# Starfish-develop/Starfish

Hardware: AMD Instinct MI355X
Metric: log-likelihood evals/sec, 4096-pixel order, batch=128 walkers (higher is better)
Workload: dtype f64; 1 GPU; cfg2: synthetic single order N_pix=4096, 8 eigenspectra, M=27, N_f=8192, 1 global + 1 local kernel, all 13 parameters thawed, batch=128 walkers per GPU; global_batch=128, units_per_gpu=128, parallelism=(order x walker) units sharded x1, one process per GPU, no data-path collective

## Files before the change

### starfish_amd/csrc/sf_chol_seq.h

```cpp
#pragma once
#include "sf_chol_host.h"
#include "sf_chol_diag.h"
#include "sf_chol_panel.h"
#include "sf_chol_wide.h"

static int sf_check_front_pad(int fp, int n) {
    if (fp != 0 && (fp != 64 || n % GT != 64)) {
        sf_set_error("potrf: front pad %d does not fit n = %d", fp, n);
        return SF_EINVAL;
    }
    return SF_OK;
}

template <class Args>
static void sf_park(Args& g, const sf_potrf_scratch& ws) {
    g.Sout = ws.T;
    g.sS = ws.sT;
    g.ldS = SF_LDT;
}
static double sf_slab_rows(int n, int row0, int nslab, int step) {
    double rows = 0.0;
    for (int i = 0; i < nslab; ++i) {
        const int r0 = row0 + i * step * GT;
        rows += (n - r0 < GT) ? n - r0 : GT;
    }
    return rows;
}
static int sf_check_grid(long long nblk) {
    if (nblk > 0x7fffffffLL) {
        sf_set_error("panel grid too large");
        return SF_EINVAL;
    }
    return SF_OK;
}

static int sf_panel_split(int k0, int pw, int fp, long long nblk) {
    return pw > 0 ? sf_split_policy(nblk, (k0 > fp ? k0 - fp : 0) / GK) : 1;
}
static int sf_panel_step(sf_panel_args g, const sf_potrf_scratch& ws, int k0, int pw, int row0, int nslab, int step, const double* Wt,
                         bool to_scratch, hipStream_t st, int region, int phase) {
    const int n = g.n, fp = g.fp, batch = ws.batch;
    g.k0 = k0;
    g.pw = pw;
    g.row0 = row0;
    g.nslab = nslab;
    g.slab_step = step;
    g.Wt = Wt;
    g.sW = ws.sW;
    if (to_scratch) {
        sf_park(g, ws);
        g.prio = 1;
    }
    const long long nblk = (long long)nslab * batch;
    SF_TRY(sf_check_grid(nblk));
    const double rows = sf_slab_rows(n, row0, nslab, step);
    const double flops_main = 2.0 * (k0 > fp ? k0 - fp : 0) * rows * pw * batch;
    const double flops_epi = (rows * pw * (double)pw + (double)GT * rows * pw) * batch;
    const int nk = (k0 > fp ? k0 - fp : 0) / GK;
    const int S = sf_panel_split(k0, pw, fp, nblk);
    void* tok;
    if (S > 1) {
        g.ksplit = S;
        g.kchunk = (nk + S - 1) / S;
        g.part = ws.part + (size_t)region * sf_split_region_tiles() * (GT * GT);
        if (phase != 2) {
            sf_prof_gemm_begin(st, flops_main, &tok);
            hipLaunchKernelGGL((k_chol_panel<false, 1>), dim3((unsigned)(nblk * S)), dim3(512), 0, st, g);
            sf_prof_gemm_end(tok);
        }
        if (phase != 1) {
            sf_prof_gemm_begin(st, flops_epi, &tok);
            if (g.rhs)
                hipLaunchKernelGGL((k_chol_panel<true, 2>), dim3((unsigned)nblk), dim3(512), 0, st, g);
            else
                hipLaunchKernelGGL((k_chol_panel<false, 2>), dim3((unsigned)nblk), dim3(512), 0, st, g);
            sf_prof_gemm_end(tok);
        }
    } else {
        sf_prof_gemm_begin(st, flops_main + flops_epi, &tok);
        if (g.rhs)
            hipLaunchKernelGGL((k_chol_panel<true, 0>), dim3((unsigned)nblk), dim3(512), 0, st, g);
        else
            hipLaunchKernelGGL((k_chol_panel<false, 0>), dim3((unsigned)nblk), dim3(512), 0, st, g);
        sf_prof_gemm_end(tok);
    }
    SF_LAUNCH_CHECK();
    return SF_OK;
}

struct sf_wide_stamps {
#ifdef SF_TUNING
    long long* t = nullptr;
    int n = 0, k[64];
#endif
};
#ifdef SF_TUNING
static int sf_wide_stamps_begin(sf_wide_stamps& w) {
    if (SF_TUNE_FLAG("SF_WIDE_STAMPS")) {
        SF_HIP(hipHostMalloc((void**)&w.t, sizeof(long long) * 16 * 64));
        for (int i = 0; i < 16 * 64; ++i) w.t[i] = 0;
    }
    return SF_OK;
}
static void sf_wide_stamps_report(sf_wide_stamps& w, hipStream_t s) {
    if (!w.t) return;
    (void)hipStreamSynchronize(s);
    fprintf(stderr, "wide launches, workgroup grid/2: k nslab | prologue | K loop | solve 1 | 2b | solve 2 | store + rhs | S load + step 4 | S store + drain | total (us)\n");
    for (int i = 0; i < w.n; ++i) {
        const long long* t = w.t + 16 * i;
        fprintf(stderr, "%2d %2d |", w.k[i] / 1000, w.k[i] % 1000);
        const int seg[8][2] = {{0, 1}, {1, 2}, {2, 3}, {3, 4}, {4, 5}, {5, 6}, {6, 7}, {7, 8}};
        for (auto& sg : seg) fprintf(stderr, " %7.1f |", (t[sg[1]] - t[sg[0]]) / 100.0);
        fprintf(stderr, " %7.1f\n", (t[8] - t[0]) / 100.0);
    }
    (void)hipHostFree(w.t);
}
#else
static int sf_wide_stamps_begin(sf_wide_stamps&) { return SF_OK; }
static void sf_wide_stamps_report(sf_wide_stamps&, hipStream_t) {}
#endif

static int sf_panel_step_w(sf_panelw_args g, const sf_potrf_scratch& ws, int k, int slab0, int nslab, int step, bool park, hipStream_t st,
                           sf_wide_stamps& stamps) {
    const int n = g.n, fp = g.fp, batch = ws.batch;
    g.k0 = k * GT;
    g.row0 = slab0 * GT;
    g.nslab = nslab;
    g.slab_step = step;
    g.Wt0 = ws.Wslot(k);
    g.Wt1 = ws.Wslot(k + 1);
    g.sW = ws.sW;
    if (park) sf_park(g, ws);
    const long long nblk = (long long)nslab * batch;
    SF_TRY(sf_check_grid(nblk));
#ifdef SF_TUNING
    if (stamps.t && stamps.n < 64) {
        stamps.k[stamps.n] = k * 1000 + nslab;
        g.stamps = stamps.t + 16 * stamps.n++;
    }
#endif
    const double rows = sf_slab_rows(n, g.row0, nslab, step);
    const double kk = g.k0 > fp ? g.k0 - fp : 0;
    const double flops = (2.0 * kk * rows * GT + 2.0 * (kk + GT) * rows * GT + 2.0 * (rows * GT * (double)GT + (double)GT * rows * GT)) * batch;
    void* tok;
    sf_prof_gemm_begin(st, flops, &tok);
    if (g.rhs)
        hipLaunchKernelGGL(k_chol_panel_w<true>, dim3((unsigned)nblk), dim3(1024), SF_PANELW_LDS, st, g);
    else
        hipLaunchKernelGGL(k_chol_panel_w<false>, dim3((unsigned)nblk), dim3(1024), SF_PANELW_LDS, st, g);
    sf_prof_gemm_end(tok);
    SF_LAUNCH_CHECK();
    return SF_OK;
}

static int sf_diag_step(const sf_potrf_scratch& ws, double* A, int lda, int64_t stride, double* rhs, int ldr, int* info, int n, int k,
                        double* Wt, int fp, hipStream_t st) {
    const int k0 = k * GT;
    const int pw = (n - k0 < GT) ? n - k0 : GT;
    return sf_launch_diag128(ws.T, ws.sT, pw, info, k0 - fp, rhs ? rhs + k0 : nullptr, ldr, A + (int64_t)k0 * lda + k0, lda, stride, Wt,
                             ws.sW, ws.batch, st, k == 0 ? fp : 0);
}

struct sf_narrow_events {
    hipEvent_t d, rest[2];
};
static int sf_narrow_step(const sf_panel_args& base, const sf_potrf_scratch& ws, sf_exec* ex, int* info, int k, double* Wt, hipStream_t c,
                          const hipStream_t gs[2], const hipEvent_t last[2], hipEvent_t* e_top, sf_narrow_events* ev) {
    const int n = base.n, fp = base.fp, nt = (n + GT - 1) / GT;
    const int k0 = k * GT;
    const int pw = (n - k0 < GT) ? n - k0 : GT;
    *ev = {};
    SF_TRY(sf_diag_step(ws, base.C, base.lda, base.sC, base.rhs, base.ldr, info, n, k, Wt, fp, c));
    if (k + 1 >= nt) return SF_OK;
    SF_TRY(sf_exec_event(ex, &ev->d));
    SF_HIP(hipEventRecord(ev->d, c));
    const int gk = (k + 1) & 1;
    if (e_top && sf_panel_split(k0, pw, fp, ws.batch) > 1) {
        if (*e_top) SF_HIP(hipStreamWaitEvent(gs[gk], *e_top, 0));
        SF_TRY(sf_panel_step(base, ws, k0, pw, (k + 1) * GT, 1, 1, Wt, true, gs[gk], 0, 1));
        hipEvent_t e_part;
        SF_TRY(sf_exec_event(ex, &e_part));
        SF_HIP(hipEventRecord(e_part, gs[gk]));
        SF_HIP(hipStreamWaitEvent(c, e_part, 0));
        SF_TRY(sf_panel_step(base, ws, k0, pw, (k + 1) * GT, 1, 1, Wt, true, c, 0, 2));
    } else {
        if (last[gk]) SF_HIP(hipStreamWaitEvent(c, last[gk], 0));
        SF_TRY(sf_panel_step(base, ws, k0, pw, (k + 1) * GT, 1, 1, Wt, true, c, 0, 0));
    }
    if (e_top) {
        SF_TRY(sf_exec_event(ex, e_top));
        SF_HIP(hipEventRecord(*e_top, c));
    }
    for (int g = 0; g < 2; ++g) {
        const int first = k + 2 + (((k + 2) & 1) != g);
        if (first >= nt) continue;
        const int cnt = (nt - 1 - first) / 2 + 1;
        SF_HIP(hipStreamWaitEvent(gs[g], ev->d, 0));
        SF_TRY(sf_panel_step(base, ws, k0, pw, first * GT, cnt, 2, Wt, false, gs[g], 1 + g, 0));
        SF_TRY(sf_exec_event(ex, &ev->rest[g]));
        SF_HIP(hipEventRecord(ev->rest[g], gs[g]));
    }
    return SF_OK;
}

static int sf_launch_potrf_v2(double* A, int n, int lda, int64_t stride, int* info, const sf_potrf_scratch& ws, double* rhs,
                              int ldr, hipStream_t s, const sf_gen_args* gen, sf_exec* ex, int fp) {
    const int batch = ws.batch;
    SF_HIP(hipMemsetAsync(info, 0, sizeof(int) * (size_t)batch, s));
    SF_TRY(sf_exec_prepare(ex));
    constexpr int G = 2;
    hipStream_t c = ex->side;
    const hipStream_t gs[G] = {s, ex->grp[0]};
    SF_TRY(sf_exec_fork(ex, s, {c, gs[1]}));

    const sf_panel_args base = sf_panel_frame<sf_panel_args>(A, n, lda, stride, rhs, ldr, gen, fp);
    const int nt = (n + GT - 1) / GT;
    SF_TRY(sf_panel_step(base, ws, 0, 0, 0, 1, 1, nullptr, true, c, 0, 0));
    hipEvent_t e_epi = nullptr;
    hipEvent_t e_rest[G] = {};
    hipEvent_t e_rest_prev[G] = {};
    for (int k = 0; k < nt; ++k) {
        for (int g = 0; g < G; ++g)
            if (e_rest_prev[g]) SF_HIP(hipStreamWaitEvent(c, e_rest_prev[g], 0));
        sf_narrow_events ev;
        SF_TRY(sf_narrow_step(base, ws, ex, info, k, ws.Wbuf(k & 1), c, gs, e_rest, &e_epi, &ev));
        for (int g = 0; g < G; ++g) {
            e_rest_prev[g] = e_rest[g];
            if (ev.rest[g]) e_rest[g] = ev.rest[g];
        }
    }
    SF_TRY(sf_exec_join(ex, s, c, {e_rest[1]}));
    return SF_OK;
}

static int sf_launch_potrf_v3(double* A, int n, int lda, int64_t stride, int* info, const sf_potrf_scratch& ws, double* rhs,
                              int ldr, hipStream_t s, const sf_gen_args* gen, sf_exec* ex, bool half, int fp) {
    const int batch = ws.batch;
    static sf_dev_once attr_once;
    SF_CHECK(sf_lds_limit_once(&attr_once, 160 * 1024, {(const void*)k_chol_panel_w<true>, (const void*)k_chol_panel_w<false>}));
    SF_HIP(hipMemsetAsync(info, 0, sizeof(int) * (size_t)batch, s));
    SF_TRY(sf_exec_prepare(ex));
    hipStream_t c = ex->side, xa = ex->side;
    SF_TRY(sf_exec_fork(ex, s, {c, xa, ex->grp[0]}));
    const int nt = (n + GT - 1) / GT;

    const sf_panel_args base = sf_panel_frame<sf_panel_args>(A, n, lda, stride, rhs, ldr, gen, fp);
    const sf_panelw_args wbase = sf_panel_frame<sf_panelw_args>(A, n, lda, stride, rhs, ldr, gen, fp);
    sf_wide_stamps stamps;
    SF_TRY(sf_wide_stamps_begin(stamps));
    auto diag = [&](int k) -> int { return sf_diag_step(ws, A, lda, stride, rhs, ldr, info, n, k, ws.Wslot(k), fp, c); };

    SF_TRY(sf_panel_step(base, ws, 0, 0, 0, 1, 1, nullptr, true, c, 0, 0));
    const hipStream_t bs[2] = {s, ex->grp[0]};
    hipEvent_t e_A = nullptr;
    hipEvent_t e_last[2] = {nullptr, nullptr};
    std::vector<hipEvent_t> readers[4];
    auto wait_readers = [&](int slot) -> int {
        for (hipEvent_t e : readers[slot]) SF_HIP(hipStreamWaitEvent(c, e, 0));
        readers[slot].clear();
        return SF_OK;
    };
    int k = 0;
    for (; k < nt; k += 2) {
        if (k + 2 >= nt) break;
        if (half && k >= (nt / 4) * 2 && k > 0) break;
        if (e_A) SF_HIP(hipStreamWaitEvent(c, e_A, 0));
        SF_TRY(wait_readers(k & 3));
        SF_TRY(diag(k));
        SF_TRY(sf_panel_step(base, ws, k * GT, GT, (k + 1) * GT, 1, 1, ws.Wslot(k), true, c, 0, 0));
        SF_TRY(wait_readers((k + 1) & 3));
        SF_TRY(diag(k + 1));
        hipEvent_t e_chain;
        SF_TRY(sf_exec_event(ex, &e_chain));
        SF_HIP(hipEventRecord(e_chain, c));
        const int na = (nt - (k + 2) < 2) ? nt - (k + 2) : 2;
        SF_HIP(hipStreamWaitEvent(xa, e_chain, 0));
        for (int g = 0; g < 2; ++g)
            if (e_last[g]) SF_HIP(hipStreamWaitEvent(xa, e_last[g], 0));
        SF_TRY(sf_panel_step_w(wbase, ws, k, k + 2, na, 1, true, xa, stamps));
        SF_TRY(sf_exec_event(ex, &e_A));
        SF_HIP(hipEventRecord(e_A, xa));
        readers[k & 3].push_back(e_A);
        readers[(k + 1) & 3].push_back(e_A);
        for (int g = 0; g < 2; ++g) {
            const int first = k + 4 + g;
            if (first >= nt) continue;
            const int cnt = (nt - 1 - first) / 2 + 1;
            SF_HIP(hipStreamWaitEvent(bs[g], e_chain, 0));
            SF_TRY(sf_panel_step_w(wbase, ws, k, first, cnt, 2, false, bs[g], stamps));
            SF_TRY(sf_exec_event(ex, &e_last[g]));
            SF_HIP(hipEventRecord(e_last[g], bs[g]));
            readers[k & 3].push_back(e_last[g]);
            readers[(k + 1) & 3].push_back(e_last[g]);
        }
    }
    for (; k < nt; ++k) {
        if (e_A) {
            SF_HIP(hipStreamWaitEvent(c, e_A, 0));
            for (int g = 0; g < 2; ++g) SF_HIP(hipStreamWaitEvent(bs[g], e_A, 0));
            e_A = nullptr;
        }
        SF_TRY(wait_readers(k & 3));
        sf_narrow_events ev;
        SF_TRY(sf_narrow_step(base, ws, ex, info, k, ws.Wslot(k), c, bs, e_last, nullptr, &ev));
        for (int g = 0; g < 2; ++g)
            if (ev.rest[g]) {
                e_last[g] = ev.rest[g];
                readers[k & 3].push_back(ev.rest[g]);
            }
    }
    SF_TRY(sf_exec_join(ex, s, c, {e_A, e_last[1]}));
    sf_wide_stamps_report(stamps, s);
    return SF_OK;
}
```

### starfish_amd/csrc/sf_chol_wide.h

```cpp
#pragma once
#include "sf_device.h"
#include "sf_chol_tile.h"
#include "sf_chol_panel.h"

#define WST (3 * GT * GK)
static constexpr size_t SF_PANELW_LDS = (3 * WST + 4 * GT) * sizeof(double);
struct sf_panelw_args {
    double* C;
    int64_t sC;
    int lda, n;
    int k0;
    int row0, nslab;
    int slab_step;
    const double* Wt0;
    const double* Wt1;
    int64_t sW;
    double* rhs;
    int ldr;
    double* Sout;
    int64_t sS;
    int ldS;
    const double* genY;
    const unsigned char* tilemap;
    int64_t sY;
    int ldy, mpad, nt128;
    int fp;
#ifdef SF_TUNING
    long long* stamps;
#endif
};
#ifdef SF_TUNING
#define SF_W_STAMP(i) do { if (g.stamps && blockIdx.x == gridDim.x / 2 && threadIdx.x == 0) g.stamps[i] = wall_clock64(); } while (0)
#else
#define SF_W_STAMP(i)
#endif

template <bool RHS>
__device__ __forceinline__ void sf_panelw_body(const sf_panelw_args& g, const int id, double* __restrict__ smw, const int tid) {
    constexpr int TM = 2, TN = 4;
    double* red = smw + 3 * WST;

    const int b = id / g.nslab;
    const int sl = id - b * g.nslab;
    const int row0 = g.row0 + sl * g.slab_step * GT;
    const int rows_here = min(GT, g.n - row0);
    const int k0 = g.k0;
    const int cfp = k0 == 0 ? g.fp : 0;

    const int lane = tid & 63;
    const int w = __builtin_amdgcn_readfirstlane(tid >> 6);
    const int wm = w & 3, wn = w >> 2;
    const int l15 = lane & 15, lq = lane >> 4;
    double* Cb = g.C + (int64_t)b * g.sC;
#define WBC(ni) ((((ni) >> 1) * GT) + wn * 32 + (((ni)&1) * 16))
    const bool wave_live = wm * 32 < rows_here;

    sf_d4 acc[TM][TN];
    SF_W_STAMP(0);
    {
        typedef __attribute__((address_space(3))) void* lds_ptr;
        const unsigned lds0 = (unsigned)(size_t)(lds_ptr)smw;
        const int grow = lane >> 3, gpos = lane & 7;
        unsigned soff[3];
        const double* sbase = sf_uniform_ptr(Cb + g.fp);
#pragma unroll
        for (int j = 0; j < 3; ++j) {
            const int G = 3 * w + j;
            const bool isA = G < 16;
            const int r = (isA ? G : G - 16) * 8 + grow;
            const int c = gpos ^ sf_swz(r);
            soff[j] = (unsigned)(((int64_t)(isA ? row0 + min(r, rows_here - 1) : k0 + r) * g.lda + 2 * c) * 8);
        }
        auto glds16 = [&](const double* sb, unsigned voff, unsigned lds_dst) {
            unsigned keep;
            asm volatile("s_mov_b32 %0, m0\n\ts_mov_b32 m0, %3\n\ts_nop 0\n\tglobal_load_lds_dwordx4 %1, %2\n\ts_mov_b32 m0, %0"
                         : "=&s"(keep)
                         : "v"(voff), "s"(sb), "s"(lds_dst)
                         : "memory");
        };
        auto gload = [&](int kt, int stage) {
#pragma unroll
            for (int j = 0; j < 3; ++j) glds16(sf_uniform_ptr(sbase + kt * GK), soff[j], lds0 + (unsigned)(stage * WST * 8 + (3 * w + j) * 1024));
        };
        auto gwait = [&]() { asm volatile("s_waitcnt vmcnt(0)" ::: "memory"); };
        const int nk = max(k0 - g.fp, 0) / GK;
        if (nk > 0) gload(0, 0);
        if (nk > 1) gload(1, 1);

        bool gen_half[2] = {false, false};
        if (g.tilemap) {
            const unsigned char* tm = g.tilemap + (int64_t)b * g.nt128 * g.nt128 + (row0 / GT) * g.nt128 + k0 / GT;
            gen_half[0] = !tm[0];
            gen_half[1] = !tm[1];
        }
#pragma unroll
        for (int hf = 0; hf < 2; ++hf) {
            if (gen_half[hf]) {
                const double* Yb = g.genY + (int64_t)b * g.sY;
                const int gr = row0 + wm * 32 + l15;
                const int gc = k0 + hf * GT + wn * 32 + l15;
#pragma unroll
                for (int mi = 0; mi < TM; ++mi)
#pragma unroll
                    for (int nn = 0; nn < 2; ++nn) acc[mi][2 * hf + nn] = (sf_d4){0.0, 0.0, 0.0, 0.0};
                for (int kk = 0; kk < g.mpad; kk += 8) {
                    double ya[2][TM], yb[2][2];
#pragma unroll
                    for (int u = 0; u < 2; ++u) {
                        const double* yk = Yb + (int64_t)(min(kk + 4 * u, g.mpad - 4) + lq) * g.ldy;
#pragma unroll
                        for (int i = 0; i < TM; ++i) ya[u][i] = yk[min(gr + i * 16, g.ldy + g.fp - 1)];
#pragma unroll
                        for (int i = 0; i < 2; ++i) yb[u][i] = gc + i * 16 >= cfp ? yk[min(gc + i * 16, g.ldy + g.fp - 1)] : 0.0;
                    }
#pragma unroll
                    for (int u = 0; u < 2; ++u) {
                        if (kk + 4 * u >= g.mpad) break;
#pragma unroll
                        for (int mi = 0; mi < TM; ++mi)
#pragma unroll
                            for (int nn = 0; nn < 2; ++nn)
                                acc[mi][2 * hf + nn] = __builtin_amdgcn_mfma_f64_16x16x4f64(ya[u][mi], yb[u][nn], acc[mi][2 * hf + nn], 0, 0, 0);
                    }
                }
            } else {
                const double* Cin = Cb + (int64_t)row0 * g.lda + k0;
#pragma unroll
                for (int mi = 0; mi < TM; ++mi)
#pragma unroll
                    for (int nn = 0; nn < 2; ++nn) {
                        const int col = WBC(2 * hf + nn) + l15;
#pragma unroll
                        for (int r = 0; r < 4; ++r) {
                            const int row = wm * 32 + mi * 16 + lq + 4 * r;
                            acc[mi][2 * hf + nn][r] = (row < rows_here && col >= cfp) ? Cin[(int64_t)row * g.lda + col] : 0.0;
                        }
                    }
            }
        }
        gwait();
        __syncthreads();
#pragma unroll
        for (int mi = 0; mi < TM; ++mi)
#pragma unroll
            for (int ni = 0; ni < TN; ++ni)
#pragma unroll
                for (int r = 0; r < 4; ++r) asm volatile("" : "+v"(acc[mi][ni][r]));
        SF_W_STAMP(1);

        const int sw = sf_swz(l15);
        const int e0 = 2 * ((2 * lq) ^ sw), e1 = 2 * ((2 * lq + 1) ^ sw);
        const int arow = (wm * 32 + l15) * GK, brow = (GT + wn * 32 + l15) * GK;
        auto frag = [&](int stage, int h, double2(&a)[TM], double2(&bb)[TN]) {
            const double* S = smw + stage * WST + (h ? e1 : e0);
#pragma unroll
            for (int i = 0; i < TM; ++i) a[i] = *(const double2*)(S + arow + i * 16 * GK);
#pragma unroll
            for (int i = 0; i < TN; ++i) bb[i] = *(const double2*)(S + brow + ((i >> 1) * GT + (i & 1) * 16) * GK);
        };
        auto mfma_part = [&](const double2(&a)[TM], const double2(&bb)[TN], auto lo_t, auto hi_t) {
            constexpr int lo = decltype(lo_t)::value, hi = decltype(hi_t)::value;
#pragma unroll
            for (int i = lo; i < hi; ++i) {
                const int y = i >> 3, mi = (i >> 2) & 1, ni = i & 3;
                acc[mi][ni] = __builtin_amdgcn_mfma_f64_16x16x4f64(y ? a[mi].y : a[mi].x, y ? bb[ni].y : bb[ni].x, acc[mi][ni], 0, 0, 1);
            }
        };
        typedef std::integral_constant<int, 0> I0;
        typedef std::integral_constant<int, 8> I8;
        typedef std::integral_constant<int, 16> I16;
        double2 a0[TM], b0[TN], a1[TM], b1[TN];
        int s0 = 0, s1 = 1, s2 = 2;
        if (nk > 0 && wave_live) frag(0, 0, a0, b0);
        for (int kt = 0; kt < nk; ++kt) {
            if (wave_live) {
                __builtin_amdgcn_s_setprio(1);
                mfma_part(a0, b0, I0(), I8());
                __builtin_amdgcn_s_setprio(0);
            }
            if (kt + 2 < nk) gload(kt + 2, s2);
            if (wave_live) {
                frag(s0, 1, a1, b1);
                __builtin_amdgcn_s_setprio(1);
                mfma_part(a0, b0, I8(), I16());
                __builtin_amdgcn_s_setprio(0);
                if (kt + 1 < nk) frag(s1, 0, a0, b0);
                __builtin_amdgcn_s_setprio(1);
                mfma_part(a1, b1, I0(), I16());
                __builtin_amdgcn_s_setprio(0);
            }
            gwait();
            __syncthreads();
            const int t = s0;
            s0 = s1;
            s1 = s2;
            s2 = t;
        }
    }

    double* Ach0 = smw;
    double* Bs = smw + 2 * GT * CLD;
    const int lr = tid >> 3, lc = (tid & 7) * 2;
    auto w_rows = [&](const double* Wt) { return Wt + (int64_t)b * g.sW + (int64_t)lr * SF_LDT + lc; };
    auto solve = [&](const double* Wt, double2 rw, auto nbtag) {
        constexpr int NB = decltype(nbtag)::value;
        const double* Wp = w_rows(Wt);
        int buf = 0;
#pragma unroll
        for (int sbi = 0; sbi < 8; ++sbi) {
            const int sb = 7 - sbi;
            double* Ach = Ach0 + ((sb >> 1) & 1) * (GT * CLD);
            if (sb == 7 && NB != 0) __syncthreads();
            if (sb & 1) {
                if (wn == (sb >> 1)) {
#pragma unroll
                    for (int nn = 0; nn < 2; ++nn)
#pragma unroll
                        for (int mi = 0; mi < TM; ++mi) {
#pragma unroll
                            for (int r = 0; r < 4; ++r)
                                Ach[(wm * 32 + mi * 16 + lq + 4 * r) * CLD + nn * 16 + l15] = acc[mi][NB + nn][r];
                            acc[mi][NB + nn] = (sf_d4){0.0, 0.0, 0.0, 0.0};
                        }
                }
            }
            {
                double* pb = Bs + buf * (GT * GLD) + lr * GLD + lc;
                pb[0] = rw.x;
                pb[1] = rw.y;
            }
            __syncthreads();
            if (sb > 0) rw = *(const double2*)(Wp + (sb - 1) * 16);
            if (sb <= 2 * wn + 1 && wave_live) {
                const double* Ab = Ach + (wm * 32 + l15) * CLD + (sb & 1) * 16 + lq;
                const double* Bb = Bs + buf * (GT * GLD) + (wn * 32 + l15) * GLD + lq;
#pragma unroll
                for (int ks = 0; ks < 4; ++ks) {
                    double a[TM], bb[2];
#pragma unroll
                    for (int i = 0; i < TM; ++i) a[i] = Ab[i * 16 * CLD + ks * 4];
#pragma unroll
                    for (int i = 0; i < 2; ++i) bb[i] = Bb[i * 16 * GLD + ks * 4];
#pragma unroll
                    for (int mi = 0; mi < TM; ++mi)
#pragma unroll
                        for (int nn = 0; nn < 2; ++nn)
                            acc[mi][NB + nn] = __builtin_amdgcn_mfma_f64_16x16x4f64(a[mi], bb[nn], acc[mi][NB + nn], 0, 0, 0);
                }
            }
            buf ^= 1;
        }
    };
    double2 rw0 = *(const double2*)(w_rows(g.Wt0) + 7 * 16);
    __syncthreads();
    SF_W_STAMP(2);
    solve(g.Wt0, rw0, std::integral_constant<int, 0>());
    SF_W_STAMP(3);
    double2 rw1 = *(const double2*)(w_rows(g.Wt1) + 7 * 16);

    {
        const double* L21 = Cb + (int64_t)(k0 + GT + lr) * g.lda + k0 + (tid & 7) * 4;
        auto l21 = [&](int q, double2& l0, double2& l1) {
            const bool real = (tid & 7) * 4 + q * 32 >= cfp;
            l0 = real ? *(const double2*)(L21 + q * 32) : make_double2(0.0, 0.0);
            l1 = real ? *(const double2*)(L21 + q * 32 + 2) : make_double2(0.0, 0.0);
        };
        double2 l0, l1, n0 = make_double2(0.0, 0.0), n1 = n0;
        l21(0, l0, l1);
#pragma unroll
        for (int q = 0; q < 4; ++q) {
            if (q + 1 < 4) l21(q + 1, n0, n1);
            double* Ach = Ach0 + (q & 1) * (GT * CLD);
            double* Bc = Bs + (q & 1) * (GT * CLD);
            if (q == 0) __syncthreads();
            if (wn == q) {
#pragma unroll
                for (int nn = 0; nn < 2; ++nn)
#pragma unroll
                    for (int mi = 0; mi < TM; ++mi)
#pragma unroll
                        for (int r = 0; r < 4; ++r)
                            Ach[(wm * 32 + mi * 16 + lq + 4 * r) * CLD + nn * 16 + l15] = acc[mi][nn][r];
            }
            {
                double* pb = Bc + lr * CLD + (tid & 7) * 4;
                pb[0] = l0.x;
                pb[1] = l0.y;
                pb[2] = l1.x;
                pb[3] = l1.y;
            }
            __syncthreads();
            if (wave_live) {
                const double* Ab = Ach + (wm * 32 + l15) * CLD + lq;
                const double* Bb = Bc + (wn * 32 + l15) * CLD + lq;
#pragma unroll
                for (int ks = 0; ks < 8; ++ks) {
                    double a[TM], bb[2];
#pragma unroll
                    for (int i = 0; i < TM; ++i) a[i] = Ab[i * 16 * CLD + ks * 4];
#pragma unroll
                    for (int i = 0; i < 2; ++i) bb[i] = Bb[i * 16 * CLD + ks * 4];
#pragma unroll
                    for (int mi = 0; mi < TM; ++mi)
#pragma unroll
                        for (int nn = 0; nn < 2; ++nn)
                            acc[mi][2 + nn] = __builtin_amdgcn_mfma_f64_16x16x4f64(a[mi], bb[nn], acc[mi][2 + nn], 0, 0, 1);
                }
            }
            l0 = n0;
            l1 = n1;
        }
    }
    SF_W_STAMP(4);
    solve(g.Wt1, rw1, std::integral_constant<int, 2>());
    SF_W_STAMP(5);
    constexpr int TLD = 130;
    const int nsb = wn == 0 ? 3 : 2;
    int sbi[3], sbj[3];
#pragma unroll
    for (int j = 0; j < 3; ++j) {
        const int t = min(wm + 4 * (wn + 4 * j), 35);
        int bi = 0;
        while ((bi + 1) * (bi + 2) / 2 <= t) ++bi;
        sbi[j] = bi;
        sbj[j] = t - bi * (bi + 1) / 2;
    }
    sf_d4 acc2[3];
    {
        const double* Sin = Cb + (int64_t)row0 * g.lda + row0;
        if (rows_here == GT) {
#pragma unroll
            for (int j = 0; j < 3; ++j)
#pragma unroll
                for (int r = 0; r < 4; ++r) {
                    const int row = 16 * sbi[j] + lq + 4 * r, col = 16 * sbj[j] + l15;
                    acc2[j][r] = Sin[(int64_t)row * g.lda + col];
                }
        } else {
#pragma unroll
            for (int j = 0; j < 3; ++j)
#pragma unroll
                for (int r = 0; r < 4; ++r) {
                    const int row = 16 * sbi[j] + lq + 4 * r, col = 16 * sbj[j] + l15;
                    acc2[j][r] = (j < nsb && row < rows_here && col < rows_here) ? Sin[(int64_t)row * g.lda + col] : 0.0;
                }
        }
    }
    double zc[TN] = {0.0, 0.0, 0.0, 0.0};
    if (RHS && g.rhs) {
        const double* z = g.rhs + (int64_t)b * g.ldr + k0;
#pragma unroll
        for (int ni = 0; ni < TN; ++ni) zc[ni] = WBC(ni) + l15 >= cfp ? z[WBC(ni) + l15] : 0.0;
    }

    {
        double* Lout = Cb + (int64_t)row0 * g.lda + k0;
#pragma unroll
        for (int mi = 0; mi < TM; ++mi)
#pragma unroll
            for (int ni = 0; ni < TN; ++ni) {
                const int col = WBC(ni) + l15;
#pragma unroll
                for (int r = 0; r < 4; ++r) {
                    const int row = wm * 32 + mi * 16 + lq + 4 * r;
                    if (row < rows_here && col >= cfp) Lout[(int64_t)row * g.lda + col] = acc[mi][ni][r];
                }
            }
        if (RHS && g.rhs) {
#pragma unroll
            for (int mi = 0; mi < TM; ++mi)
#pragma unroll
                for (int r = 0; r < 4; ++r) {
                    double v = 0.0;
#pragma unroll
                    for (int ni = 0; ni < TN; ++ni) v = __builtin_fma(acc[mi][ni][r], zc[ni], v);
                    v += __shfl_xor(v, 1);
                    v += __shfl_xor(v, 2);
                    v += __shfl_xor(v, 4);
                    v += __shfl_xor(v, 8);
                    if (l15 == 0) red[wn * GT + wm * 32 + mi * 16 + lq + 4 * r] = v;
                }
        }
    }

    SF_W_STAMP(6);
    {
        double* Ts = smw;
#pragma unroll
        for (int half = 0; half < 2; ++half) {
            __syncthreads();
#pragma unroll
            for (int nn = 0; nn < 2; ++nn)
#pragma unroll
                for (int mi = 0; mi < TM; ++mi)
#pragma unroll
                    for (int r = 0; r < 4; ++r)
                        Ts[(wm * 32 + mi * 16 + lq + 4 * r) * TLD + wn * 32 + nn * 16 + l15] = acc[mi][2 * half + nn][r];
            __syncthreads();
#pragma unroll
            for (int j = 0; j < 3; ++j) {
                if (j >= nsb) continue;
                const double* Pa = Ts + (sbi[j] * 16 + l15) * TLD + lq;
                const double* Pb = Ts + (sbj[j] * 16 + l15) * TLD + lq;
#pragma unroll 8
                for (int ks = 0; ks < GT / 4; ++ks)
                    acc2[j] = __builtin_amdgcn_mfma_f64_16x16x4f64(Pa[ks * 4], Pb[ks * 4], acc2[j], 0, 0, 1);
            }
        }
        SF_W_STAMP(7);
        const bool parked = g.Sout && sl == 0;
        double* So = parked ? g.Sout + (int64_t)b * g.sS : Cb + (int64_t)row0 * g.lda + row0;
        const int ldo = parked ? g.ldS : g.lda;
        if (rows_here == GT) {
#pragma unroll
            for (int j = 0; j < 2; ++j)
#pragma unroll
                for (int r = 0; r < 4; ++r) {
                    const int row = 16 * sbi[j] + lq + 4 * r, col = 16 * sbj[j] + l15;
                    So[(int64_t)row * ldo + col] = acc2[j][r];
                }
            if (nsb == 3) {
#pragma unroll
                for (int r = 0; r < 4; ++r) {
                    const int row = 16 * sbi[2] + lq + 4 * r, col = 16 * sbj[2] + l15;
                    So[(int64_t)row * ldo + col] = acc2[2][r];
                }
            }
        } else {
#pragma unroll
            for (int j = 0; j < 3; ++j) {
                if (j >= nsb) continue;
#pragma unroll
                for (int r = 0; r < 4; ++r) {
                    const int row = 16 * sbi[j] + lq + 4 * r, col = 16 * sbj[j] + l15;
                    if (row < rows_here && col < rows_here) So[(int64_t)row * ldo + col] = acc2[j][r];
                }
            }
        }
    }
    if (RHS && g.rhs) {
        if (tid < rows_here)
            g.rhs[(int64_t)b * g.ldr + row0 + tid] -= (red[tid] + red[GT + tid]) + (red[2 * GT + tid] + red[3 * GT + tid]);
    }
#ifdef SF_TUNING
    if (g.stamps) {
        __syncthreads();
        asm volatile("s_waitcnt vmcnt(0)" ::: "memory");
        SF_W_STAMP(8);
    }
#endif
#undef WBC
}
template <bool RHS>
__global__ __launch_bounds__(1024) void k_chol_panel_w(sf_panelw_args g) {
    extern __shared__ __attribute__((aligned(16))) double smw[];
    sf_panelw_body<RHS>(g, sf_xcd_remap(blockIdx.x, gridDim.x), smw, threadIdx.x);
}
#undef SF_W_STAMP
#undef WST
```

Before: 2768 evals/s.

## Restage wide panel solve in 32-column chunks and interleave L stores with SYRK MFMAs

The triangular solve now stages W in four 32-column chunks instead of eight 16-column blocks. This halves the number of barriers in the solve loop, and the next chunk and the L21 tiles are prefetched while the current MFMAs run. The L21 update loop is software-pipelined: it dumps and stages the next tile before the MFMAs on the current one, and it prefetches the second solve's W chunks. Global stores of the L panel are moved out of a standalone loop and interleaved between the step-4 SYRK MFMA groups, with schedule barriers to hide store latency. Tuning-only timestamps are added around step 4, and the scheme costs extra registers for prefetched data and more complex LDS buffer parity.

```diff
diff --git a/starfish_amd/csrc/sf_chol_seq.h b/starfish_amd/csrc/sf_chol_seq.h
--- a/starfish_amd/csrc/sf_chol_seq.h
+++ b/starfish_amd/csrc/sf_chol_seq.h
@@ -112,6 +112,14 @@
         const int seg[8][2] = {{0, 1}, {1, 2}, {2, 3}, {3, 4}, {4, 5}, {5, 6}, {6, 7}, {7, 8}};
         for (auto& sg : seg) fprintf(stderr, " %7.1f |", (t[sg[1]] - t[sg[0]]) / 100.0);
         fprintf(stderr, " %7.1f\n", (t[8] - t[0]) / 100.0);
+    }
+    fprintf(stderr, "step 4 of the same launches: k nslab | half 0: dump | wait for S | MFMA | half 1: dump | wait for S | MFMA (us)\n");
+    for (int i = 0; i < w.n; ++i) {
+        const long long* t = w.t + 16 * i;
+        fprintf(stderr, "%2d %2d |", w.k[i] / 1000, w.k[i] % 1000);
+        const int seg[6][2] = {{6, 9}, {9, 10}, {10, 11}, {11, 12}, {12, 13}, {13, 14}};
+        for (auto& sg : seg) fprintf(stderr, " %7.2f |", (t[sg[1]] - t[sg[0]]) / 100.0);
+        fprintf(stderr, "\n");
     }
     (void)hipHostFree(w.t);
 }
diff --git a/starfish_amd/csrc/sf_chol_wide.h b/starfish_amd/csrc/sf_chol_wide.h
--- a/starfish_amd/csrc/sf_chol_wide.h
+++ b/starfish_amd/csrc/sf_chol_wide.h
@@ -201,78 +201,98 @@
     double* Ach0 = smw;
     double* Bs = smw + 2 * GT * CLD;
     const int lr = tid >> 3, lc = (tid & 7) * 2;
-    auto w_rows = [&](const double* Wt) { return Wt + (int64_t)b * g.sW + (int64_t)lr * SF_LDT + lc; };
-    auto solve = [&](const double* Wt, double2 rw, auto nbtag) {
+    auto w_rows = [&](const double* Wt) { return Wt + (int64_t)b * g.sW + (int64_t)lr * SF_LDT + 2 * lc; };
+    auto w_chunk = [&](const double* Wp, int c, double2& r0, double2& r1) {
+        r0 = *(const double2*)(Wp + c * 32);
+        r1 = *(const double2*)(Wp + c * 32 + 2);
+    };
+    auto stage4 = [&](double* pb, double2 r0, double2 r1) {
+        pb[0] = r0.x;
+        pb[1] = r0.y;
+        pb[2] = r1.x;
+        pb[3] = r1.y;
+    };
+    auto solve = [&](const double* Wt, double2 (&rw)[4], auto nbtag, auto&& ahead) {
         constexpr int NB = decltype(nbtag)::value;
         const double* Wp = w_rows(Wt);
-        int buf = 0;
-#pragma unroll
-        for (int sbi = 0; sbi < 8; ++sbi) {
-            const int sb = 7 - sbi;
-            double* Ach = Ach0 + ((sb >> 1) & 1) * (GT * CLD);
-            if (sb == 7 && NB != 0) __syncthreads();
-            if (sb & 1) {
-                if (wn == (sb >> 1)) {
-#pragma unroll
-                    for (int nn = 0; nn < 2; ++nn)
-#pragma unroll
-                        for (int mi = 0; mi < TM; ++mi) {
-#pragma unroll
-                            for (int r = 0; r < 4; ++r)
-                                Ach[(wm * 32 + mi * 16 + lq + 4 * r) * CLD + nn * 16 + l15] = acc[mi][NB + nn][r];
-                            acc[mi][NB + nn] = (sf_d4){0.0, 0.0, 0.0, 0.0};
-                        }
-                }
-            }
-            {
-                double* pb = Bs + buf * (GT * GLD) + lr * GLD + lc;
-                pb[0] = rw.x;
-                pb[1] = rw.y;
-            }
+        auto stage = [&](int c, double2 r0, double2 r1) {
+            double* Ach = Ach0 + (c & 1) * (GT * CLD);
+            if (wn == c) {
+#pragma unroll
+                for (int nn = 0; nn < 2; ++nn)
+#pragma unroll
+                    for (int mi = 0; mi < TM; ++mi) {
+#pragma unroll
+                        for (int r = 0; r < 4; ++r)
+                            Ach[(wm * 32 + mi * 16 + lq + 4 * r) * CLD + nn * 16 + l15] = acc[mi][NB + nn][r];
+                        acc[mi][NB + nn] = (sf_d4){0.0, 0.0, 0.0, 0.0};
+                    }
+            }
+            stage4(Bs + (c & 1) * (GT * CLD) + lr * CLD + 2 * lc, r0, r1);
+        };
+        stage(3, rw[0], rw[1]);
+        w_chunk(Wp, 1, rw[0], rw[1]);
+#pragma unroll
+        for (int ci = 0; ci < 4; ++ci) {
+            const int c = 3 - ci;
             __syncthreads();
-            if (sb > 0) rw = *(const double2*)(Wp + (sb - 1) * 16);
-            if (sb <= 2 * wn + 1 && wave_live) {
-                const double* Ab = Ach + (wm * 32 + l15) * CLD + (sb & 1) * 16 + lq;
-                const double* Bb = Bs + buf * (GT * GLD) + (wn * 32 + l15) * GLD + lq;
-#pragma unroll
-                for (int ks = 0; ks < 4; ++ks) {
-                    double a[TM], bb[2];
-#pragma unroll
-                    for (int i = 0; i < TM; ++i) a[i] = Ab[i * 16 * CLD + ks * 4];
-#pragma unroll
-                    for (int i = 0; i < 2; ++i) bb[i] = Bb[i * 16 * GLD + ks * 4];
-#pragma unroll
-                    for (int mi = 0; mi < TM; ++mi)
-#pragma unroll
-                        for (int nn = 0; nn < 2; ++nn)
-                            acc[mi][NB + nn] = __builtin_amdgcn_mfma_f64_16x16x4f64(a[mi], bb[nn], acc[mi][NB + nn], 0, 0, 0);
-                }
-            }
-            buf ^= 1;
+            if (c == 3) {
+                stage(2, rw[2], rw[3]);
+                w_chunk(Wp, 0, rw[2], rw[3]);
+            }
+            if (c == 2) stage(1, rw[0], rw[1]);
+            if (c == 1) {
+                stage(0, rw[2], rw[3]);
+            }
+            if (c <= 1) ahead(c);
+#pragma unroll
+            for (int sb = 2 * c + 1; sb >= 2 * c; --sb) {
+                if (sb <= 2 * wn + 1 && wave_live) {
+                    const double* Ab = Ach0 + (c & 1) * (GT * CLD) + (wm * 32 + l15) * CLD + (sb & 1) * 16 + lq;
+                    const double* Bb = Bs + (c & 1) * (GT * CLD) + (wn * 32 + l15) * CLD + (sb & 1) * 16 + lq;
+#pragma unroll
+                    for (int ks = 0; ks < 4; ++ks) {
+                        double a[TM], bb[2];
+#pragma unroll
+                        for (int i = 0; i < TM; ++i) a[i] = Ab[i * 16 * CLD + ks * 4];
+#pragma unroll
+                        for (int i = 0; i < 2; ++i) bb[i] = Bb[i * 16 * CLD + ks * 4];
+#pragma unroll
+                        for (int mi = 0; mi < TM; ++mi)
+#pragma unroll
+                            for (int nn = 0; nn < 2; ++nn)
+                                acc[mi][NB + nn] = __builtin_amdgcn_mfma_f64_16x16x4f64(a[mi], bb[nn], acc[mi][NB + nn], 0, 0, 0);
+                    }
+                }
+            }
         }
     };
-    double2 rw0 = *(const double2*)(w_rows(g.Wt0) + 7 * 16);
+    double2 rw[4];
+    w_chunk(w_rows(g.Wt0), 3, rw[0], rw[1]);
+    w_chunk(w_rows(g.Wt0), 2, rw[2], rw[3]);
     __syncthreads();
     SF_W_STAMP(2);
-    solve(g.Wt0, rw0, std::integral_constant<int, 0>());
+    const double* L21 = Cb + (int64_t)(k0 + GT + lr) * g.lda + k0 + 2 * lc;
+    auto l21 = [&](int q, double2& l0, double2& l1) {
+        const bool real = 2 * lc + q * 32 >= cfp;
+        l0 = real ? *(const double2*)(L21 + q * 32) : make_double2(0.0, 0.0);
+        l1 = real ? *(const double2*)(L21 + q * 32 + 2) : make_double2(0.0, 0.0);
+    };
+    double2 n0 = make_double2(0.0, 0.0), n1 = n0;
+    auto stage_l21 = [&](int q, double2 r0, double2 r1) { stage4(Bs + ((q & 1) ^ 1) * (GT * CLD) + lr * CLD + 2 * lc, r0, r1); };
+    solve(g.Wt0, rw, std::integral_constant<int, 0>(), [&](int c) {
+        if (c == 1) {
+            l21(0, n0, n1);
+        } else {
+            stage_l21(0, n0, n1);
+            l21(1, n0, n1);
+        }
+    });
     SF_W_STAMP(3);
-    double2 rw1 = *(const double2*)(w_rows(g.Wt1) + 7 * 16);
 
     {
-        const double* L21 = Cb + (int64_t)(k0 + GT + lr) * g.lda + k0 + (tid & 7) * 4;
-        auto l21 = [&](int q, double2& l0, double2& l1) {
-            const bool real = (tid & 7) * 4 + q * 32 >= cfp;
-            l0 = real ? *(const double2*)(L21 + q * 32) : make_double2(0.0, 0.0);
-            l1 = real ? *(const double2*)(L21 + q * 32 + 2) : make_double2(0.0, 0.0);
-        };
-        double2 l0, l1, n0 = make_double2(0.0, 0.0), n1 = n0;
-        l21(0, l0, l1);
-#pragma unroll
-        for (int q = 0; q < 4; ++q) {
-            if (q + 1 < 4) l21(q + 1, n0, n1);
-            double* Ach = Ach0 + (q & 1) * (GT * CLD);
-            double* Bc = Bs + (q & 1) * (GT * CLD);
-            if (q == 0) __syncthreads();
+        auto dump = [&](int q) {
+            double* Ach = Ach0 + ((q & 1) ^ 1) * (GT * CLD);
             if (wn == q) {
 #pragma unroll
                 for (int nn = 0; nn < 2; ++nn)
@@ -282,17 +302,21 @@
                         for (int r = 0; r < 4; ++r)
                             Ach[(wm * 32 + mi * 16 + lq + 4 * r) * CLD + nn * 16 + l15] = acc[mi][nn][r];
             }
-            {
-                double* pb = Bc + lr * CLD + (tid & 7) * 4;
-                pb[0] = l0.x;
-                pb[1] = l0.y;
-                pb[2] = l1.x;
-                pb[3] = l1.y;
-            }
+        };
+        dump(0);
+#pragma unroll
+        for (int q = 0; q < 4; ++q) {
             __syncthreads();
+            if (q + 1 < 4) {
+                dump(q + 1);
+                stage_l21(q + 1, n0, n1);
+                if (q + 2 < 4) l21(q + 2, n0, n1);
+            }
+            if (q == 2) w_chunk(w_rows(g.Wt1), 3, rw[0], rw[1]);
+            if (q == 3) w_chunk(w_rows(g.Wt1), 2, rw[2], rw[3]);
             if (wave_live) {
-                const double* Ab = Ach + (wm * 32 + l15) * CLD + lq;
-                const double* Bb = Bc + (wn * 32 + l15) * CLD + lq;
+                const double* Ab = Ach0 + ((q & 1) ^ 1) * (GT * CLD) + (wm * 32 + l15) * CLD + lq;
+                const double* Bb = Bs + ((q & 1) ^ 1) * (GT * CLD) + (wn * 32 + l15) * CLD + lq;
 #pragma unroll
                 for (int ks = 0; ks < 8; ++ks) {
                     double a[TM], bb[2];
@@ -307,12 +331,10 @@
                             acc[mi][2 + nn] = __builtin_amdgcn_mfma_f64_16x16x4f64(a[mi], bb[nn], acc[mi][2 + nn], 0, 0, 1);
                 }
             }
-            l0 = n0;
-            l1 = n1;
         }
     }
     SF_W_STAMP(4);
-    solve(g.Wt1, rw1, std::integral_constant<int, 2>());
+    solve(g.Wt1, rw, std::integral_constant<int, 2>(), [](int) {});
     SF_W_STAMP(5);
     constexpr int TLD = 130;
     const int nsb = wn == 0 ? 3 : 2;
@@ -353,19 +375,13 @@
         for (int ni = 0; ni < TN; ++ni) zc[ni] = WBC(ni) + l15 >= cfp ? z[WBC(ni) + l15] : 0.0;
     }
 
+    double* Lout = Cb + (int64_t)row0 * g.lda + k0;
+    auto store_L = [&](int half, int s) {
+        const int mi = s >> 3, ni = 2 * half + ((s >> 2) & 1), r = s & 3;
+        const int row = wm * 32 + mi * 16 + lq + 4 * r, col = WBC(ni) + l15;
+        if (row < rows_here && col >= cfp) Lout[(int64_t)row * g.lda + col] = acc[mi][ni][r];
+    };
     {
-        double* Lout = Cb + (int64_t)row0 * g.lda + k0;
-#pragma unroll
-        for (int mi = 0; mi < TM; ++mi)
-#pragma unroll
-            for (int ni = 0; ni < TN; ++ni) {
-                const int col = WBC(ni) + l15;
-#pragma unroll
-                for (int r = 0; r < 4; ++r) {
-                    const int row = wm * 32 + mi * 16 + lq + 4 * r;
-                    if (row < rows_here && col >= cfp) Lout[(int64_t)row * g.lda + col] = acc[mi][ni][r];
-                }
-            }
         if (RHS && g.rhs) {
 #pragma unroll
             for (int mi = 0; mi < TM; ++mi)
@@ -397,15 +413,34 @@
                     for (int r = 0; r < 4; ++r)
                         Ts[(wm * 32 + mi * 16 + lq + 4 * r) * TLD + wn * 32 + nn * 16 + l15] = acc[mi][2 * half + nn][r];
             __syncthreads();
+#ifdef SF_TUNING
+            if (g.stamps) {
+                SF_W_STAMP(9 + 3 * half);
+#pragma unroll
+                for (int j = 0; j < 3; ++j)
+#pragma unroll
+                    for (int r = 0; r < 4; ++r) asm volatile("" : "+v"(acc2[j][r]));
+                SF_W_STAMP(10 + 3 * half);
+            }
+#endif
 #pragma unroll
             for (int j = 0; j < 3; ++j) {
                 if (j >= nsb) continue;
                 const double* Pa = Ts + (sbi[j] * 16 + l15) * TLD + lq;
                 const double* Pb = Ts + (sbj[j] * 16 + l15) * TLD + lq;
-#pragma unroll 8
-                for (int ks = 0; ks < GT / 4; ++ks)
-                    acc2[j] = __builtin_amdgcn_mfma_f64_16x16x4f64(Pa[ks * 4], Pb[ks * 4], acc2[j], 0, 0, 1);
-            }
+#pragma unroll
+                for (int u = 0; u < GT / 32; ++u) {
+#pragma unroll
+                    for (int ks = 8 * u; ks < 8 * u + 8; ++ks)
+                        acc2[j] = __builtin_amdgcn_mfma_f64_16x16x4f64(Pa[ks * 4], Pb[ks * 4], acc2[j], 0, 0, 1);
+                    if (4 * j + u < 8) {
+                        store_L(half, 2 * (4 * j + u));
+                        store_L(half, 2 * (4 * j + u) + 1);
+                    }
+                    __builtin_amdgcn_sched_barrier(0);
+                }
+            }
+            SF_W_STAMP(11 + 3 * half);
         }
         SF_W_STAMP(7);
         const bool parked = g.Sout && sl == 0;
```

After: 2802 evals/s (median of 6 runs). +1.2%, better.
